# hongsukchoi/Pose2Mesh_RELEASE

Hardware: AMD Instinct MI355X
Metric: SMPL meshes/sec fwd+bwd at batch 256 (higher is better)
Workload: dtype f32 (emulated on the BF16 matrix pipe: every operand as 3 exact bf16 slices = 24-bit significands, 6 slice products per fp32 product, fp32 accumulate)

## Files before the change

pose2mesh_release_amd/csrc/gemm.hip:

```cpp
#include <cstdlib>
#include <type_traits>

#include "p2m_split.h"

namespace p2m {

constexpr int BM = 128;
constexpr int BK = 32;
constexpr int AS_LD = BK + 1;

struct GemmArgs {
  const float* A[3];
  const float* Bm;
  const float* bias;
  const float* addend;
  const float* act_scale;
  const float* act_shift;
  int act_relu;
  int pair_out;
  float* C[3];
  float* stats;
  long M;
  int nplanesA, Ka, a0_shift;
  int N, Nc;
  int ntm, ntn;
  const int* ids;
  int nset, V, tps, compact;
  const float* row_w;
  const unsigned short* Bx;
  int Npad, Ktot;
  const unsigned* a_amax;
  const unsigned* b_amax;
  int a_bits;
  unsigned* amax_out;
  const float* in_scale;
  const float* in_shift;
};

__device__ __forceinline__ bool tile_of_block(int bid, int ntm, int ntn, int& mt, int& nt) {
  int xcd = bid & 7;
  int slot = bid >> 3;
  nt = slot % ntn;
  mt = (slot / ntn) * 8 + xcd;
  return mt < ntm;
}

constexpr int ROWTAB_WORDS = 2 * BM + 2;
__device__ __forceinline__ void rows_weights_fill(const GemmArgs& g, int* rowtab, int i, int t) {
  float* wtab = reinterpret_cast<float*>(rowtab + BM);
  const float w = (i < g.nset) ? g.row_w[i] : 0.f;
  wtab[t] = w;
  float s = w;
#pragma unroll
  for (int o = 32; o > 0; o >>= 1) s += __shfl_xor(s, o);
  if ((t & 63) == 0) wtab[BM + (t >> 6)] = s;
}

template <int BN, bool EXTRA, bool ROWS>
__device__ __forceinline__ void gemm_epilogue(const GemmArgs& g, floatx16 (&acc)[2][BN / 64], float* smem,
                                              const int* rowtab, int mt, long m0, int n0, int rs_i0, int wm, int wn,
                                              int l31, int lhi, int descale = 0) {
  constexpr int WTN = BN / 2;
  constexpr int TN = WTN / 32;
  constexpr int TM = 2;
  float bias_v[TN], sc_v[TN], sh_v[TN];
  int ncol[TN];
#pragma unroll
  for (int j = 0; j < TN; j++) {
    ncol[j] = n0 + wn * WTN + j * 32 + l31;
    bias_v[j] = (g.bias != nullptr && ncol[j] < g.N) ? g.bias[ncol[j]] : 0.f;
    sc_v[j] = (g.act_scale != nullptr && ncol[j] < g.N) ? g.act_scale[ncol[j]] : 1.f;
    sh_v[j] = (g.act_scale != nullptr && ncol[j] < g.N) ? g.act_shift[ncol[j]] : 0.f;
  }
  float csum[TN];
  float vmax = 0.f;
  const bool wst = ROWS && g.row_w != nullptr && g.stats != nullptr;
  const float* wtab = reinterpret_cast<const float*>(rowtab + BM);
#pragma unroll
  for (int j = 0; j < TN; j++) csum[j] = 0.f;
#pragma unroll
  for (int i = 0; i < TM; i++)
#pragma unroll
    for (int j = 0; j < TN; j++) {
      const int n = ncol[j];
      const int q = n / g.Nc;
      const int c = n - q * g.Nc;
      float* Cq = (n < g.N) ? g.C[q] : nullptr;
#pragma unroll
      for (int r = 0; r < 16; r++) {
        const int ml = wm * 64 + i * 32 + (r & 3) + 8 * (r >> 2) + 4 * lhi;
        long row = ROWS ? (long)rowtab[ml] : m0 + ml;
        const bool rok = ROWS ? (row >= 0) : (row < g.M);
        float v = __builtin_ldexpf(acc[i][j][r], descale) + bias_v[j];
        if (g.act_scale != nullptr) v = fmaf(v, sc_v[j], sh_v[j]);
        if (g.act_relu) v = fmaxf(v, 0.f);
        if (EXTRA && g.addend != nullptr && rok && Cq != nullptr) v += g.addend[row * g.N + n];
        acc[i][j][r] = rok ? v : 0.f;
        if (!(EXTRA && g.pair_out) && rok && Cq != nullptr) {
#ifdef P2M_PL_ABL_NOSTORE
          if (v == 12345.678f)
#endif
          Cq[row * g.Nc + c] = v;
          csum[j] += wst ? wtab[ml] * v : v;
          vmax = fmaxf(vmax, amax_abs(v));
        }
        if ((r & 3) == 3) __builtin_amdgcn_sched_barrier(0);
      }
      if (EXTRA && g.pair_out && Cq != nullptr) {
#pragma unroll
        for (int r = 0; r < 16; r += 2) {
          long row = m0 + wm * 64 + i * 32 + (r & 3) + 8 * (r >> 2) + 4 * lhi;
          if (row < g.M) {
            const float pv = acc[i][j][r] + acc[i][j][r + 1];
            Cq[(row >> 1) * g.Nc + c] = pv;
            vmax = fmaxf(vmax, amax_abs(pv));
          }
        }
      }
    }
  if (g.amax_out != nullptr) amax_commit(g.amax_out, vmax);
  if (g.stats == nullptr) return;

  float* red = smem;
  long rows_valid = ROWS ? (long)(g.nset - rs_i0) : g.M - m0;
  if (rows_valid > BM) rows_valid = BM;
#pragma unroll
  for (int j = 0; j < TN; j++) {
    csum[j] += __shfl_xor(csum[j], 32);
    if (lhi == 0) red[wm * BN + wn * WTN + j * 32 + l31] = csum[j];
  }
  __syncthreads();
  float cm2[TN];
#pragma unroll
  for (int j = 0; j < TN; j++) {
    const int cl = wn * WTN + j * 32 + l31;
    const float tot = red[cl] + red[BN + cl];
    const float mean = tot / (wst ? wtab[BM] + wtab[BM + 1] : (float)rows_valid);
    float m2 = 0.f;
#pragma unroll
    for (int i = 0; i < TM; i++)
#pragma unroll
      for (int r = 0; r < 16; r++) {
        const int ml = wm * 64 + i * 32 + (r & 3) + 8 * (r >> 2) + 4 * lhi;
        float d = acc[i][j][r] - mean;
        if (ROWS ? (rowtab[ml] >= 0) : (m0 + ml < g.M)) m2 += wst ? wtab[ml] * d * d : d * d;
      }
    m2 += __shfl_xor(m2, 32);
    cm2[j] = m2;
    csum[j] = tot;
  }
  __syncthreads();
#pragma unroll
  for (int j = 0; j < TN; j++)
    if (lhi == 0) red[wm * BN + wn * WTN + j * 32 + l31] = cm2[j];
  __syncthreads();
  if (wm == 0 && lhi == 0) {
#pragma unroll
    for (int j = 0; j < TN; j++) {
      const int cl = wn * WTN + j * 32 + l31;
      const int n = n0 + cl;
      if (n < g.N) {
        float* st = g.stats + (long)mt * 2 * g.N;
        st[n] = csum[j];
        st[g.N + n] = red[cl] + red[BN + cl];
      }
    }
  }
}

template <int BN, int KB, bool EXTRA, bool ROWS = false>
__global__ __launch_bounds__(256, 2) void k_gemm_planes(GemmArgs g) {
  constexpr int WTN = BN / 2;
  constexpr int TN = WTN / 32;
  constexpr int TM = 2;
  constexpr int LDA = KB + 1;
  constexpr int APASS = BM * KB / 4 / 256;
  constexpr int AROWS = 256 / (KB / 4);
  constexpr int BPASS = KB * BN / 4 / 256;
  constexpr int BROWS = 256 / (BN / 4);
  __shared__ float smem[2 * BM * LDA + 2 * KB * BN + (ROWS ? ROWTAB_WORDS : 0)];
  float* As = smem;
  float* Bs = smem + 2 * BM * LDA;
  int* rowtab = reinterpret_cast<int*>(smem + 2 * BM * LDA + 2 * KB * BN);

  int mt, nt;
  if (!tile_of_block(blockIdx.x, g.ntm, g.ntn, mt, nt)) return;
  const long m0 = (long)mt * BM;
  const int n0 = nt * BN;
  const int t = threadIdx.x;
  const int rs_b = ROWS ? mt / g.tps : 0;
  const int rs_i0 = ROWS ? (mt - rs_b * g.tps) * BM : 0;
  if (ROWS && t < BM) {
    const int i = rs_i0 + t;
    rowtab[t] = (i < g.nset) ? rs_b * g.V + g.ids[i] : -1;
    if (g.row_w != nullptr) rows_weights_fill(g, rowtab, i, t);
  }
  const int lane = t & 63, wave = t >> 6;
  const int wm = wave >> 1, wn = wave & 1;
  const int l31 = lane & 31, lhi = lane >> 5;

  floatx16 acc[TM][TN];
#pragma unroll
  for (int i = 0; i < TM; i++)
#pragma unroll
    for (int j = 0; j < TN; j++)
#pragma unroll
      for (int r = 0; r < 16; r++) acc[i][j][r] = 0.f;

  const int cpp = g.Ka / KB;
  const int nchunks = g.nplanesA * cpp;

  float4 ra[APASS];
  float4 rb[BPASS];
  const int a_row = t / (KB / 4), a_k4 = (t % (KB / 4)) * 4;
  const int b_row = t / (BN / 4), b_c4 = (t % (BN / 4)) * 4;
  long rs_full[ROWS ? APASS : 1], rs_comp[ROWS ? APASS : 1];
  if (ROWS) {
#pragma unroll
    for (int ps = 0; ps < APASS; ps++) {
      const int i = rs_i0 + ps * AROWS + a_row;
      if (i < g.nset) {
        rs_full[ps] = (long)rs_b * g.V + g.ids[i];
        rs_comp[ps] = (long)rs_b * g.nset + i;
      } else {
        rs_full[ps] = -1;
        rs_comp[ps] = -1;
      }
    }
  }

  auto load_chunk = [&](int kc) {
    const int p = kc / cpp;
    const int k0 = (kc - p * cpp) * KB;
    const float* Ap = g.A[p];
    const int sh = (p == 0) ? g.a0_shift : 0;
#pragma unroll
    for (int ps = 0; ps < APASS; ps++) {
      if (ROWS) {
        const long r = (p == 0 || !g.compact) ? rs_full[ps] : rs_comp[ps];
        if (r >= 0)
          ra[ps] = *reinterpret_cast<const float4*>(Ap + (r >> sh) * g.Ka + k0 + a_k4);
        else
          ra[ps] = make_float4(0.f, 0.f, 0.f, 0.f);
      } else {
        long r = m0 + ps * AROWS + a_row;
        if (r < g.M)
          ra[ps] = *reinterpret_cast<const float4*>(Ap + (r >> sh) * g.Ka + k0 + a_k4);
        else
          ra[ps] = make_float4(0.f, 0.f, 0.f, 0.f);
      }
    }
    const float* Bp = g.Bm + (long)(p * g.Ka + k0) * g.N;
#pragma unroll
    for (int ps = 0; ps < BPASS; ps++) {
      int kr = ps * BROWS + b_row;
      int n = n0 + b_c4;
      if (n < g.N)
        rb[ps] = *reinterpret_cast<const float4*>(Bp + (long)kr * g.N + n);
      else
        rb[ps] = make_float4(0.f, 0.f, 0.f, 0.f);
    }
  };
  auto store_chunk = [&](int buf) {
// ... 185 lines not shown
      for (int q = 0; q < NS; q++) *reinterpret_cast<u32x4*>(d + q * BN * LDX) = b[q];
    };
    const int last = n - 1;
#pragma unroll
    for (int i = 0; i < NST; i++) load_chunk(i < last ? i : last, ra[i], rb[i]);
#pragma unroll
    for (int i = 0; i < AHEAD; i++) {
      if (i < n) store_chunk(i, ra[i], rb[i]);
      load_chunk(NST + i < last ? NST + i : last, ra[i], rb[i]);
    }
    lds_barrier();
    int kc = 0;
    for (; kc + (NST - 1) + AHEAD + NST < n; kc += NST) {
#pragma unroll
      for (int i = 0; i < NST; i++) {
        store_chunk(kc + i + AHEAD, ra[(i + AHEAD) % NST], rb[(i + AHEAD) % NST]);
        load_chunk(kc + i + AHEAD + NST, ra[(i + AHEAD) % NST], rb[(i + AHEAD) % NST]);
        lds_barrier();
      }
    }
    for (; kc < n; kc += NST) {
#pragma unroll
      for (int i = 0; i < NST; i++) {
        if (kc + i < n) {
          if (kc + i + AHEAD < n) store_chunk(kc + i + AHEAD, ra[(i + AHEAD) % NST], rb[(i + AHEAD) % NST]);
          if (kc + i + AHEAD + NST < n) load_chunk(kc + i + AHEAD + NST, ra[(i + AHEAD) % NST], rb[(i + AHEAD) % NST]);
          lds_barrier();
        }
      }
    }
  } else {
    frag_t fa[NBUF - 1][NS][TM], fb[NBUF - 1][NS][TN];
    auto read_frags = [&](int kc, frag_t (&a)[NS][TM], frag_t (&b)[NS][TN]) {
      const int buf = kc % NBUF;
      const unsigned short* as = As + buf * A_BUF + (wm * 64 + l31) * LDX + lhi * 8;
      const unsigned short* bs = Bs + buf * B_BUF + (wn * WTN + l31) * LDX + lhi * 8;
#pragma unroll
      for (int sl = 0; sl < NS; sl++) {
#pragma unroll
        for (int i = 0; i < TM; i++)
          a[sl][i] = __builtin_bit_cast(frag_t, *reinterpret_cast<const u32x4*>(as + (sl * BM + i * 32) * LDX));
#pragma unroll
        for (int j = 0; j < TN; j++)
          b[sl][j] = __builtin_bit_cast(frag_t, *reinterpret_cast<const u32x4*>(bs + (sl * BN + j * 32) * LDX));
      }
    };
    auto mfmas = [&](const frag_t (&a)[NS][TM], const frag_t (&b)[NS][TN]) {
#define P2M_PAIR(SA, SB)                                                                       \
  _Pragma("unroll") for (int i = 0; i < TM; i++) _Pragma("unroll") for (int j = 0; j < TN; j++) \
      acc[i][j] = slice_mfma<NS>(a[SA][i], b[SB][j], acc[i][j]);
#ifdef P2M_PL_ABL_NOMFMA
      if constexpr (NS == 3) {
        P2M_PAIR(0, 0)
        for (int sl = 1; sl < NS; sl++)
          for (int i = 0; i < TM; i++) for (int j = 0; j < TN; j++) { asm volatile("" :: "v"(a[sl][i])); asm volatile("" :: "v"(b[sl][j])); }
      } else
#endif
      if constexpr (NS == 3) {
        P2M_PAIR(2, 0)
        P2M_PAIR(0, 2)
        P2M_PAIR(1, 1)
        P2M_PAIR(1, 0)
        P2M_PAIR(0, 1)
        P2M_PAIR(0, 0)
      } else {
        P2M_PAIR(1, 0)
        P2M_PAIR(0, 1)
        P2M_PAIR(0, 0)
      }
#undef P2M_PAIR
    };
    lds_barrier();
    for (int kc = 0; kc < n; kc++) {
      read_frags(kc, fa[0], fb[0]);
      mfmas(fa[0], fb[0]);
      lds_barrier();
    }
  }
  __syncthreads();
  if (!producer) {
    gemm_epilogue<BN, EXTRA, ROWS>(g, acc, smem, rowtab, mt, m0, n0, rs_i0, wm, wn, l31, lhi, descale);
  } else {
    if (g.stats != nullptr) {
      __syncthreads();
      __syncthreads();
      __syncthreads();
    }
  }
}

#ifdef P2M_K1_TRACE
__device__ unsigned long long g_k1_tr[4096][4];
#define P2M_K1T(ev)                                                                      \
  do {                                                                                   \
    if (threadIdx.x == 0 && blockIdx.x < 4096) g_k1_tr[blockIdx.x][ev] = __builtin_amdgcn_s_memtime(); \
  } while (0)
#else
#define P2M_K1T(ev) do { } while (0)
#endif

template <int BN, bool EXTRA, int NS, int KP>
__global__ __launch_bounds__(256, 2) void k_gemm_rows_k1(GemmArgs g) {
  typedef typename SliceFrag<NS>::type frag_t;
  constexpr bool ROWS = true;
  constexpr int WTN = BN / 2;
  constexpr int TN = WTN / 32;
  constexpr int TM = 2;
  constexpr int LDX = KP + 8;
  constexpr int TPR = KP / 4;
  constexpr int RPS = 256 / TPR;
  constexpr int NSW = BM / RPS;
  constexpr int KSTEPS = KP / 16;
  constexpr int A_IMG = NS * BM * LDX;
  static_assert(KP == 64 || KP == 32, "pass width");
  static_assert(A_IMG / 2 >= 2 * BN, "the epilogue's reduction buffer lives in the image");
  __shared__ __attribute__((aligned(16))) float smem[A_IMG / 2 + ROWTAB_WORDS];
  __shared__ __attribute__((aligned(16))) float actco[2 * 256];
  unsigned short* As = reinterpret_cast<unsigned short*>(smem);
  int* rowtab = reinterpret_cast<int*>(smem + A_IMG / 2);

  int mt, nt;
  if (!tile_of_block(blockIdx.x, g.ntm, g.ntn, mt, nt)) return;
  P2M_K1T(0);
  const int t = threadIdx.x;
  const long m0 = (long)mt * BM;
  const int n0 = nt * BN;
  const int rs_b = mt / g.tps;
  const int rs_i0 = (mt - rs_b * g.tps) * BM;
  const int lane = t & 63, wave = t >> 6;
  const int wm = wave >> 1, wn = wave & 1;
  const int l31 = lane & 31, lhi = lane >> 5;
  const int npass = g.Ka / KP;
  const bool in_act = g.in_scale != nullptr;
  const bool live = n0 + wn * WTN < g.N;
  float a_sc = 1.f;
  int descale = 0;
  if (NS == 2) {
    const int sa = slice_scale_exp(*g.a_amax, g.a_bits);
    a_sc = exp2_int(sa);
    descale = -(sa + slice_scale_exp(*g.b_amax, 0));
  }

  int rt_row = -1;
  float rt_w = 0.f, co_sc = 0.f, co_sh = 0.f;
  if (t < BM) {
    const int i = rs_i0 + t;
    if (i < g.nset) {
      rt_row = rs_b * g.V + g.ids[i];
      if (g.row_w != nullptr) rt_w = g.row_w[i];
    }
  }
  if (in_act && t < g.Ka) {
    co_sc = g.in_scale[t];
    co_sh = g.in_shift[t];
  }

  const int a_g = t / TPR;
  const int a_row = KP == 64 ? a_g : (((a_g & 1) << 2) | ((a_g >> 1) & 3) | ((a_g >> 3) << 3));
  const int a_k4 = (t % TPR) * 4;
  const long sbase0 = (((long)rs_b * g.V) >> g.a0_shift) * g.Ka;
  unsigned voff[NSW];
#pragma unroll
  for (int ps = 0; ps < NSW; ps++) {
    int i = rs_i0 + ps * RPS + a_row;
    if (i >= g.nset) i = g.nset - 1;
    voff[ps] = (unsigned)((((g.ids[i] >> g.a0_shift) * g.Ka) + a_k4) * 4);
  }
  f32x4 ra[2][NSW];
  auto load_pass = [&](int p, f32x4 (&a)[NSW]) {
    const char* Ab = reinterpret_cast<const char*>(g.A[0] + sbase0 + p * KP);
#pragma unroll
    for (int ps = 0; ps < NSW; ps++) a[ps] = *reinterpret_cast<const f32x4*>(Ab + voff[ps]);
  };
  auto store_pass = [&](int p, f32x4 (&a)[NSW]) {
    if (in_act) {
      const f32x4 sc = *reinterpret_cast<const f32x4*>(&actco[p * KP + a_k4]);
      const f32x4 sh = *reinterpret_cast<const f32x4*>(&actco[256 + p * KP + a_k4]);
#pragma unroll
      for (int ps = 0; ps < NSW; ps++)
#pragma unroll
        for (int e = 0; e < 4; e++) a[ps][e] = fmaxf(fmaf(a[ps][e], sc[e], sh[e]), 0.f);
    }
#pragma unroll
    for (int ps = 0; ps < NSW; ps++) {
      u32x2 sl[NS];
      split_pack4<NS>(a[ps][0], a[ps][1], a[ps][2], a[ps][3], a_sc, sl);
      unsigned short* d = As + (ps * RPS + a_row) * LDX + a_k4;
#pragma unroll
      for (int q = 0; q < NS; q++) *reinterpret_cast<u32x2*>(d + q * BM * LDX) = sl[q];
    }
  };

  load_pass(0, ra[0]);
  if (npass > 1) load_pass(1, ra[1]);

  const long bx_slice = (long)g.Npad * 16;
  const int nsteps = g.Ka / 16;
  unsigned bx_voff[TN];
// ... 623 lines not shown
    if constexpr (NS == 3) {
      P2M_PAIR(2, 0)
      P2M_PAIR(0, 2)
      P2M_PAIR(1, 1)
      P2M_PAIR(1, 0)
      P2M_PAIR(0, 1)
      P2M_PAIR(0, 0)
    } else {
      P2M_PAIR(1, 0)
      P2M_PAIR(0, 1)
      P2M_PAIR(0, 0)
    }
#undef P2M_PAIR
    P2M_TNT(kc, 2);
    (void)kc;
  };
  auto lds_barrier = [] { asm volatile("s_waitcnt lgkmcnt(0)\n\ts_barrier" ::: "memory"); };

  for (int sb = 0; sb < nsamp; sb++) {
  if (nst > 0) {
    if (producer) {
      load_ids(0, id0);
      load_ids(1, id1);
      load_stage(0, x0, id0, true_type{});
      load_ids(2, id0);
      load_stage(nst > 1 ? 1 : 0, x1, id1, true_type{});
      load_ids(3, id1);
      store_stage(0, 0, x0, true_type{});
      load_stage(nst > 2 ? 2 : nst - 1, x0, id0, true_type{});
      load_ids(4, id0);
      lds_barrier();
      int kc = 0;
      for (; kc + 5 < nst; kc += 2) {
        P2M_TNT(kc + 1, 0);
        store_stage(1, kc + 1, x1, false_type{});
        load_stage(kc + 3, x1, id1, false_type{});
        load_ids(kc + 5, id1);
        P2M_TNT(kc + 1, 3);
        lds_barrier();
        P2M_TNT(kc + 2, 0);
        store_stage(0, kc + 2, x0, false_type{});
        load_stage(kc + 4, x0, id0, false_type{});
        load_ids(kc + 6, id0);
        P2M_TNT(kc + 2, 3);
        lds_barrier();
      }
      for (; kc < nst; kc += 2) {
        if (kc + 1 < nst) store_stage(1, kc + 1, x1, true_type{});
        if (kc + 3 < nst) {
          load_stage(kc + 3, x1, id1, true_type{});
          load_ids(kc + 5, id1);
        }
        lds_barrier();
        if (kc + 1 < nst) {
          if (kc + 2 < nst) store_stage(0, kc + 2, x0, true_type{});
          if (kc + 4 < nst) {
            load_stage(kc + 4, x0, id0, true_type{});
            load_ids(kc + 6, id0);
          }
          lds_barrier();
        }
      }
    } else {
      lds_barrier();
      for (int kc = 0; kc < nst; kc++) {
        P2M_TNT(kc, 0);
        compute(kc & 1, kc);
        P2M_TNT(kc, 3);
        lds_barrier();
      }
    }
  }
  srcb += samp_bytes;
  }
  __syncthreads();

  float* Pc = g.P + (long)chunk * g.Ktot * g.N;
  if (!producer) {
#pragma unroll
    for (int i = 0; i < TM; i++)
#pragma unroll
      for (int j = 0; j < TN; j++) {
        const int n = n0 + wn * WTN + j * 32 + l31;
        float old[16];
#pragma unroll
        for (int r = 0; r < 16; r++) {
          const int krow = kk0 + wm * 64 + i * 32 + (r & 3) + 8 * (r >> 2) + 4 * lhi;
          old[r] = (g.accum && krow < g.Ktot && n < g.N) ? Pc[(long)krow * g.N + n] : 0.f;
        }
#pragma unroll
        for (int r = 0; r < 16; r++) {
          const int krow = kk0 + wm * 64 + i * 32 + (r & 3) + 8 * (r >> 2) + 4 * lhi;
          if (krow < g.Ktot && n < g.N) Pc[(long)krow * g.N + n] = __builtin_ldexpf(acc[i][j][r], descale) + old[r];
        }
      }
  }
  if (kt == 0 && g.Pdb != nullptr) {
    float* red = smem;
    if (producer && !is_a && (st >> 2) < BN / 4) *reinterpret_cast<f32x4*>(red + rq * BN + c4 * 4) = dbs;
    __syncthreads();
    if (t < BN) {
      const float sum = red[t] + red[BN + t] + red[2 * BN + t] + red[3 * BN + t];
      if (n0 + t < g.N) g.Pdb[(long)chunk * g.N + n0 + t] = sum;
    }
  }
}

__global__ void k_naive_gemm_tn(TnArgs g) {
  int o = blockIdx.x * blockDim.x + threadIdx.x;
  const int chunk = blockIdx.y;
  const long r_begin = (long)chunk * g.chunk_rows;
  long r_end = r_begin + g.chunk_rows;
  if (r_end > g.M) r_end = g.M;
  const int nout = g.Ktot * g.N;
  if (o < nout) {
    int kk = o / g.N, n = o - kk * g.N;
    int p = kk / g.Ka, k = kk - p * g.Ka;
    const float* Ap = g.A[p];
    int sh = p == 0 ? g.a0_shift : 0;
    float acc = 0.f;
    const int q = n / g.Gc;
    const float* Gq = g.G[q] + (n - q * g.Gc);
    for (long r = r_begin; r < r_end; r++) acc = fmaf(Ap[(r >> sh) * g.Ka + k], Gq[r * g.Gc], acc);
    g.P[(long)chunk * nout + o] = g.accum ? g.P[(long)chunk * nout + o] + acc : acc;
  }
  if (g.Pdb != nullptr && o < g.N) {
    float s = 0.f;
    const int q = o / g.Gc;
    const float* Gq = g.G[q] + (o - q * g.Gc);
    for (long r = r_begin; r < r_end; r++) s += Gq[r * g.Gc];
    g.Pdb[(long)chunk * g.N + o] = s;
  }
}

__global__ void k_weight_pack(const float* __restrict__ W, float* __restrict__ Wt, float* __restrict__ W2,
                              float* __restrict__ W3, int Fout, int Fin, int K) {
  long idx = (long)blockIdx.x * blockDim.x + threadIdx.x;
  long tot = (long)Fout * Fin * K;
  if (idx >= tot) return;
  int fout = (int)(idx % Fout);
  long kk = idx / Fout;
  int k = (int)(kk / Fin), fin = (int)(kk % Fin);
  float v = W[(long)fout * Fin * K + (long)fin * K + k];
  Wt[idx] = v;
  if (W2) W2[(long)fout * Fin * K + kk] = v;
  if (W3) W3[((long)k * Fout + fout) * Fin + fin] = v;
}

__global__ __launch_bounds__(256) void k_transpose_tiled(const float* __restrict__ W, float* __restrict__ Wt, int R, int C) {
  __shared__ float tile[64][65];
  const int r0 = blockIdx.y * 64, c0 = blockIdx.x * 64;
  const int tq = threadIdx.x & 15, ty = threadIdx.x >> 4;
  const bool vec = (C & 3) == 0 && (R & 3) == 0;
#pragma unroll
  for (int p = 0; p < 4; p++) {
    const int r = r0 + ty + 16 * p, c = c0 + 4 * tq;
    if (r < R) {
      if (vec && c + 3 < C) {
        const float4 v = *reinterpret_cast<const float4*>(W + (long)r * C + c);
        tile[ty + 16 * p][4 * tq] = v.x; tile[ty + 16 * p][4 * tq + 1] = v.y;
        tile[ty + 16 * p][4 * tq + 2] = v.z; tile[ty + 16 * p][4 * tq + 3] = v.w;
      } else {
        for (int e = 0; e < 4; e++)
          if (c + e < C) tile[ty + 16 * p][4 * tq + e] = W[(long)r * C + c + e];
      }
    }
  }
  __syncthreads();
#pragma unroll
  for (int p = 0; p < 4; p++) {
    const int c = c0 + ty + 16 * p, r = r0 + 4 * tq;
    if (c < C) {
      if (vec && r + 3 < R) {
        float4 v;
        v.x = tile[4 * tq][ty + 16 * p]; v.y = tile[4 * tq + 1][ty + 16 * p];
        v.z = tile[4 * tq + 2][ty + 16 * p]; v.w = tile[4 * tq + 3][ty + 16 * p];
// ... 317 lines not shown
extern "C" int p2m_gemm_planes(const float* A0, const float* A1, const float* A2, int32_t nplanesA, int32_t Ka,
                               int32_t a0_shift, const float* Bm, const void* Bsplit, int32_t arith,
                               const void* a_amax, int32_t a_bits, const float* bias,
                               const float* addend, float* C0, float* C1, float* C2, int32_t nplanesC, int32_t Nc,
                               int32_t pair_out, int64_t M, float* stats, const float* act_scale,
                               const float* act_shift, int32_t act_relu, void* amax_out, void* stream) {
  P2M_CHECK_ARG(nplanesA >= 1 && nplanesA <= 3 && nplanesC >= 1 && nplanesC <= 3, "plane count must be 1..3");
  P2M_CHECK_ARG(arith == P2M_ARITH_F32 || arith == P2M_ARITH_BF16X3 || arith == P2M_ARITH_F16X2, "unknown arithmetic");
  P2M_CHECK_ARG((act_scale == nullptr) == (act_shift == nullptr), "act_scale / act_shift must both be given or both NULL");
  P2M_CHECK_ARG(!((act_scale || act_relu) && (stats || pair_out)), "fused activation excludes stats and pair_out");
  P2M_CHECK_ARG(A0 && Bm && C0 && Ka > 0 && Nc > 0, "null pointer or empty shape");
  P2M_CHECK_ARG(a0_shift == 0 || a0_shift == 1, "a0_shift must be 0 or 1");
  if (M <= 0) return P2M_OK;
  GemmArgs g;
  g.A[0] = A0; g.A[1] = A1; g.A[2] = A2;
  g.C[0] = C0; g.C[1] = C1; g.C[2] = C2;
  for (int p = 0; p < nplanesA; p++) P2M_CHECK_ARG(g.A[p] != nullptr, "missing A plane");
  for (int p = 0; p < nplanesC; p++) P2M_CHECK_ARG(g.C[p] != nullptr, "missing C plane");
  P2M_CHECK_ARG((addend == nullptr && !pair_out) || nplanesC == 1, "addend / pair_out need a single output plane");
  P2M_CHECK_ARG(!(pair_out && stats), "pair_out and stats are mutually exclusive");
  g.Bm = Bm; g.bias = bias; g.addend = addend; g.pair_out = pair_out; g.stats = stats; g.M = M;
  g.act_scale = act_scale; g.act_shift = act_shift; g.act_relu = act_relu;
  g.nplanesA = nplanesA; g.Ka = Ka; g.a0_shift = a0_shift;
  g.N = nplanesC * Nc; g.Nc = Nc;
  g.ids = nullptr; g.nset = 0; g.V = 0; g.tps = 0; g.compact = 0; g.row_w = nullptr;
  g.Bx = nullptr; g.Npad = 0; g.Ktot = 0;
  g.a_amax = g.b_amax = nullptr; g.a_bits = 0;
  g.amax_out = static_cast<unsigned*>(amax_out);
  g.in_scale = g.in_shift = nullptr;
  hipStream_t s = (hipStream_t)stream;
  const bool mfma_ok = (Ka % BK == 0) && (g.N % 32 == 0) && (Nc % 32 == 0);
  if (!mfma_ok) {
    P2M_CHECK_ARG(!pair_out, "pair_out needs the MFMA path (Ka % 32 == 0, N % 32 == 0)");
    P2M_CHECK_ARG(!amax_out, "amax_out needs the MFMA path (Ka % 32 == 0, N % 32 == 0)");
    long tot = M * g.N;
    g.ntm = g.ntn = 0;
    hipLaunchKernelGGL(k_naive_gemm_planes, dim3(cdiv(tot, 256)), dim3(256), 0, s, g);
    if (stats) {
      P2M_CHECK_ARG(nplanesC == 1, "stats need a single output plane");
      hipLaunchKernelGGL(k_naive_tile_stats, dim3(cdiv(M, BM)), dim3(64), 0, s, C0, stats, (long)M, g.N);
    }
    return check_launch("gemm_planes(naive)");
  }
  if (arith != P2M_ARITH_F32) {
    P2M_CHECK_ARG(Bsplit != nullptr, "the slice arithmetics need the pre-split weight (p2m_weight_split)");
    P2M_CHECK_ARG(arith != P2M_ARITH_F16X2 || a_amax != nullptr, "P2M_ARITH_F16X2 needs the amax word of the A planes");
    g.Bx = static_cast<const unsigned short*>(Bsplit);
    g.Npad = cdiv(g.N, 128) * 128;
    g.Ktot = nplanesA * Ka;
    if (arith == P2M_ARITH_F16X2) {
      g.a_amax = static_cast<const unsigned*>(a_amax);
      g.a_bits = a_bits;
      g.b_amax = weight_amax_word(Bsplit, arith, g.Npad, g.Ktot);
    }
  }
  g.ntm = cdiv(M, BM);
  launch_gemm_planes<false>(g, addend != nullptr || pair_out, s);
  return check_launch("gemm_planes");
}

extern "C" int p2m_gemm_planes_rows(p2m_graph_t gh, int32_t row_set, int32_t B, const float* A0, const float* A1,
                                    const float* A2, int32_t nplanesA, int32_t Ka, int32_t a0_shift,
                                    int32_t planes_compact, const float* Bm, const void* Bsplit, int32_t arith,
                                    const void* a_amax, int32_t a_bits, const float* bias,
                                    const float* addend, float* C, int32_t N, float* stats, const float* act_scale,
                                    const float* act_shift, int32_t act_relu, void* amax_out, const float* in_scale,
                                    const float* in_shift, void* stream) {
  P2M_CHECK_ARG(gh && A0 && Bm && C, "null pointer");
  P2M_CHECK_ARG((in_scale == nullptr) == (in_shift == nullptr), "in_scale / in_shift must both be given or both NULL");
  P2M_CHECK_ARG(in_scale == nullptr || (arith != P2M_ARITH_F32 && Ka <= 256),
                "activation on load exists in the slice arithmetics only, for Ka <= 256");
  P2M_CHECK_ARG(arith == P2M_ARITH_F32 || arith == P2M_ARITH_BF16X3 || arith == P2M_ARITH_F16X2, "unknown arithmetic");
  P2M_CHECK_ARG(arith == P2M_ARITH_F32 || Bsplit != nullptr, "the slice arithmetics need the pre-split weight (p2m_weight_split)");
  P2M_CHECK_ARG(arith != P2M_ARITH_F16X2 || a_amax != nullptr, "P2M_ARITH_F16X2 needs the amax word of the A planes");
  P2M_CHECK_ARG((act_scale == nullptr) == (act_shift == nullptr), "act_scale / act_shift must both be given or both NULL");
  P2M_CHECK_ARG(!((act_scale || act_relu) && stats), "fused activation excludes stats");
  P2M_CHECK_ARG(row_set_valid(row_set), "row_set must be 1 (real), 2 (fake), 3 (paired real) or 4 (paired fake)");
  P2M_CHECK_ARG(nplanesA >= 1 && nplanesA <= 3, "plane count must be 1..3");
  P2M_CHECK_ARG(Ka > 0 && Ka % BK == 0 && N > 0 && N % 32 == 0, "Ka and N must be positive multiples of 32");
  P2M_CHECK_ARG(a0_shift == 0 || a0_shift == 1, "a0_shift must be 0 or 1");
  const Graph& gr = *reinterpret_cast<const Graph*>(gh);
  const RowSet rs = row_set_of(gr, row_set);
  if (B <= 0 || rs.n == 0) return P2M_OK;
  GemmArgs g;
  g.A[0] = A0; g.A[1] = A1; g.A[2] = A2;
  for (int p = 0; p < nplanesA; p++) P2M_CHECK_ARG(g.A[p] != nullptr, "missing A plane");
  g.C[0] = C; g.C[1] = nullptr; g.C[2] = nullptr;
  g.Bm = Bm; g.bias = bias; g.addend = addend; g.pair_out = 0; g.stats = stats;
  g.act_scale = act_scale; g.act_shift = act_shift; g.act_relu = act_relu;
  g.nplanesA = nplanesA; g.Ka = Ka; g.a0_shift = a0_shift; g.N = N; g.Nc = N;
  g.ids = rs.ids; g.nset = rs.n; g.V = rs.V; g.tps = cdiv(rs.n, BM); g.compact = planes_compact;
  g.row_w = (stats != nullptr && row_set == 2) ? gr.fake_wts : nullptr;
  g.Bx = arith == P2M_ARITH_F32 ? nullptr : static_cast<const unsigned short*>(Bsplit);
  g.Npad = cdiv(N, 128) * 128;
  g.Ktot = nplanesA * Ka;
  g.a_amax = g.b_amax = nullptr; g.a_bits = 0;
  if (arith == P2M_ARITH_F16X2) {
    g.a_amax = static_cast<const unsigned*>(a_amax);
    g.a_bits = a_bits;
    g.b_amax = weight_amax_word(Bsplit, arith, g.Npad, g.Ktot);
  }
  g.amax_out = static_cast<unsigned*>(amax_out);
  g.in_scale = in_scale; g.in_shift = in_shift;
  g.M = (long)B * g.tps * BM;
  g.ntm = B * g.tps;
  launch_gemm_planes<true>(g, addend != nullptr, (hipStream_t)stream);
  return check_launch("gemm_planes_rows");
}

extern "C" int32_t p2m_rows_tiles_per_sample(p2m_graph_t gh, int32_t row_set) {
  if (!gh || !row_set_valid(row_set)) return 0;
  const Graph& gr = *reinterpret_cast<const Graph*>(gh);
  return cdiv(row_set_of(gr, row_set).n, BM);
}

static int gemm_tn_impl(const float* A0, const float* A1, const float* A2, int32_t nplanesA, int32_t Ka,
                        int32_t a0_shift, const float* G0, const float* G1, const float* G2, int32_t nplanesG,
                        int32_t Gc, int64_t M, int64_t chunk_rows, float* P, float* Pdb, int32_t arith,
                        const void* a_amax, int32_t a_bits, const void* g_amax, int32_t g_bits, int32_t accumulate,
                        void* stream);
extern "C" int p2m_gemm_tn(const float* A0, const float* A1, const float* A2, int32_t nplanesA, int32_t Ka,
                           int32_t a0_shift, const float* G0, const float* G1, const float* G2, int32_t nplanesG,
                           int32_t Gc, int64_t M, int64_t chunk_rows, float* P, float* Pdb, int32_t arith,
                           const void* a_amax, int32_t a_bits, const void* g_amax, int32_t g_bits, void* stream) {
  return gemm_tn_impl(A0, A1, A2, nplanesA, Ka, a0_shift, G0, G1, G2, nplanesG, Gc, M, chunk_rows, P, Pdb, arith, a_amax,
                      a_bits, g_amax, g_bits, 0, stream);
}
extern "C" int p2m_gemm_tn_acc(const float* A, int32_t Ka, const float* G, int32_t N, int64_t M, float* P, int32_t arith,
                               const void* a_amax, const void* g_amax, void* stream) {
  const int64_t chunk_rows = ((M + 31) / 32) * 32;
  return gemm_tn_impl(A, nullptr, nullptr, 1, Ka, 0, G, nullptr, nullptr, 1, N, M, chunk_rows > 0 ? chunk_rows : 32, P,
                      nullptr, arith, a_amax, 0, g_amax, 0, 1, stream);
}
static int gemm_tn_impl(const float* A0, const float* A1, const float* A2, int32_t nplanesA, int32_t Ka,
                        int32_t a0_shift, const float* G0, const float* G1, const float* G2, int32_t nplanesG,
                        int32_t Gc, int64_t M, int64_t chunk_rows, float* P, float* Pdb, int32_t arith,
                        const void* a_amax, int32_t a_bits, const void* g_amax, int32_t g_bits, int32_t accumulate,
                        void* stream) {
  P2M_CHECK_ARG(nplanesA >= 1 && nplanesA <= 3 && nplanesG >= 1 && nplanesG <= 3, "plane count must be 1..3");
  P2M_CHECK_ARG(arith == P2M_ARITH_F32 || arith == P2M_ARITH_BF16X3 || arith == P2M_ARITH_F16X2, "unknown arithmetic");
  P2M_CHECK_ARG(arith != P2M_ARITH_F16X2 || (a_amax && g_amax), "P2M_ARITH_F16X2 needs the amax words of both operands");
  const int N = nplanesG * Gc;
  P2M_CHECK_ARG(A0 && G0 && P && Ka > 0 && Gc > 0 && chunk_rows > 0, "null pointer or empty shape");
  P2M_CHECK_ARG(a0_shift == 0 || a0_shift == 1, "a0_shift must be 0 or 1");
  if (M <= 0) return P2M_OK;
  TnArgs g;
  g.A[0] = A0; g.A[1] = A1; g.A[2] = A2;
  for (int p = 0; p < nplanesA; p++) P2M_CHECK_ARG(g.A[p] != nullptr, "missing A plane");
  g.G[0] = G0; g.G[1] = G1; g.G[2] = G2; g.Gc = Gc;
  for (int p = 0; p < nplanesG; p++) P2M_CHECK_ARG(g.G[p] != nullptr, "missing G plane");
  g.P = P; g.Pdb = Pdb; g.M = M; g.chunk_rows = chunk_rows;
  g.nplanesA = nplanesA; g.Ka = Ka; g.a0_shift = a0_shift; g.Ktot = nplanesA * Ka; g.N = N;
  g.ids = nullptr; g.nset = 0; g.V = 0; g.splits = 1; g.compact = 0;
  g.a_amax = static_cast<const unsigned*>(a_amax); g.g_amax = static_cast<const unsigned*>(g_amax);
  g.a_bits = a_bits; g.g_bits = g_bits;
  g.a_scale = g.a_shift = nullptr;
  const int nchunks = cdiv(M, chunk_rows);
  g.nchunks = nchunks;
  g.accum = accumulate;
  P2M_CHECK_ARG(!accumulate || nchunks == 1, "accumulation needs the whole reduction in one chunk");
  hipStream_t s = (hipStream_t)stream;
  const bool mfma_ok = (Ka % 4 == 0) && (N % 32 == 0) && (Gc % 4 == 0) && (g.Ktot >= 32);
  if (!mfma_ok) {
    g.nkt = g.ntn = 0;
    int nout = g.Ktot * N;
    if (nout < N) nout = N;
// ... 133 lines not shown
```

Measured before the change: 6248.

## Restructure GEMM epilogue with 32-bit offsets, prefetched addends and fewer barriers

Rewrites the GEMM epilogue to work in groups of four rows. Row offsets come from a vectorised rowtab read and are held as 32-bit byte offsets from a per-sample base pointer. Addend loads are double-buffered one group ahead, waves whose column range lies entirely outside N skip the work, and the stats reduction uses two separate LDS buffers so one barrier is dropped. The TN kernel also skips the old-value reload when not accumulating. In exchange, pointer offsets are limited to 32 bits (enforced by a new argument check), register pressure rises from copying the accumulators into val, and the producer barrier count must stay matched to the consumer's.

Measured after the change: 6447 (median of 6 runs). +3.2%, better.

```diff
diff --git a/pose2mesh_release_amd/csrc/gemm.hip b/pose2mesh_release_amd/csrc/gemm.hip
--- a/pose2mesh_release_amd/csrc/gemm.hip
+++ b/pose2mesh_release_amd/csrc/gemm.hip
@@ -56,6 +56,19 @@
   if ((t & 63) == 0) wtab[BM + (t >> 6)] = s;
 }
 
+template <bool ROWS>
+__device__ __forceinline__ void epi_group_rows(const int* rowtab, long m0, long M, int ml0, int (&rl)[4]) {
+  if (ROWS) {
+    const u32x4 rt = *reinterpret_cast<const u32x4*>(rowtab + ml0);
+#pragma unroll
+    for (int e = 0; e < 4; e++) rl[e] = (int)rt[e];
+  } else {
+#pragma unroll
+    for (int e = 0; e < 4; e++) rl[e] = (m0 + ml0 + e < M) ? ml0 + e : -1;
+  }
+}
+
+constexpr int EPI_BARRIERS = 2;
 template <int BN, bool EXTRA, bool ROWS>
 __device__ __forceinline__ void gemm_epilogue(const GemmArgs& g, floatx16 (&acc)[2][BN / 64], float* smem,
                                               const int* rowtab, int mt, long m0, int n0, int rs_i0, int wm, int wn,
@@ -63,109 +76,214 @@
   constexpr int WTN = BN / 2;
   constexpr int TN = WTN / 32;
   constexpr int TM = 2;
-  float bias_v[TN], sc_v[TN], sh_v[TN];
-  int ncol[TN];
-#pragma unroll
-  for (int j = 0; j < TN; j++) {
-    ncol[j] = n0 + wn * WTN + j * 32 + l31;
-    bias_v[j] = (g.bias != nullptr && ncol[j] < g.N) ? g.bias[ncol[j]] : 0.f;
-    sc_v[j] = (g.act_scale != nullptr && ncol[j] < g.N) ? g.act_scale[ncol[j]] : 1.f;
-    sh_v[j] = (g.act_scale != nullptr && ncol[j] < g.N) ? g.act_shift[ncol[j]] : 0.f;
-  }
+  constexpr int NG = TM * 4;
+  const int wnu = __builtin_amdgcn_readfirstlane(wn);
+  const bool live = n0 + wnu * WTN < g.N;
+  const bool wst = ROWS && g.row_w != nullptr && g.stats != nullptr;
+  const float* wtab = reinterpret_cast<const float*>(rowtab + BM);
+  const int mlw = wm * 64 + 4 * lhi;
   float csum[TN];
   float vmax = 0.f;
-  const bool wst = ROWS && g.row_w != nullptr && g.stats != nullptr;
-  const float* wtab = reinterpret_cast<const float*>(rowtab + BM);
 #pragma unroll
   for (int j = 0; j < TN; j++) csum[j] = 0.f;
+  float val[TM][TN][16];
 #pragma unroll
   for (int i = 0; i < TM; i++)
 #pragma unroll
+    for (int j = 0; j < TN; j++)
+#pragma unroll
+      for (int r = 0; r < 16; r++) val[i][j][r] = acc[i][j][r];
+
+  if (live) {
+    float bias_v[TN], sc_v[TN], sh_v[TN];
+    bool cok[TN];
+    unsigned c4[TN];
+    char* Cb[TN];
+    const bool pair = EXTRA && !ROWS && g.pair_out;
+    const long rowbase = ROWS ? (long)(mt / g.tps) * g.V : m0;
+    const int rowbase32 = (int)rowbase;
+    const unsigned pitch = (unsigned)g.Nc * 4u;
+#pragma unroll
     for (int j = 0; j < TN; j++) {
-      const int n = ncol[j];
-      const int q = n / g.Nc;
-      const int c = n - q * g.Nc;
-      float* Cq = (n < g.N) ? g.C[q] : nullptr;
-#pragma unroll
-      for (int r = 0; r < 16; r++) {
-        const int ml = wm * 64 + i * 32 + (r & 3) + 8 * (r >> 2) + 4 * lhi;
-        long row = ROWS ? (long)rowtab[ml] : m0 + ml;
-        const bool rok = ROWS ? (row >= 0) : (row < g.M);
-        float v = __builtin_ldexpf(acc[i][j][r], descale) + bias_v[j];
-        if (g.act_scale != nullptr) v = fmaf(v, sc_v[j], sh_v[j]);
-        if (g.act_relu) v = fmaxf(v, 0.f);
-        if (EXTRA && g.addend != nullptr && rok && Cq != nullptr) v += g.addend[row * g.N + n];
-        acc[i][j][r] = rok ? v : 0.f;
-        if (!(EXTRA && g.pair_out) && rok && Cq != nullptr) {
+      const int nu = n0 + wnu * WTN + j * 32;
+      const int n = nu + l31;
+      cok[j] = n < g.N;
+      bias_v[j] = (g.bias != nullptr && cok[j]) ? g.bias[n] : 0.f;
+      sc_v[j] = (g.act_scale != nullptr && cok[j]) ? g.act_scale[n] : 1.f;
+      sh_v[j] = (g.act_scale != nullptr && cok[j]) ? g.act_shift[n] : 0.f;
+      const int q = (nu >= g.Nc ? 1 : 0) + (nu >= 2 * g.Nc ? 1 : 0);
+      float* const Cq = q == 0 ? g.C[0] : (q == 1 ? g.C[1] : g.C[2]);
+      Cb[j] = reinterpret_cast<char*>(Cq + (pair ? rowbase >> 1 : rowbase) * g.Nc);
+      c4[j] = (unsigned)(n - q * g.Nc) * 4u;
+    }
+    const char* const Ab = reinterpret_cast<const char*>(g.addend + (EXTRA && g.addend != nullptr ? rowbase * g.Nc : 0));
+    constexpr unsigned NOROW = 0xFFFFFFFFu;
+
+    auto row_offsets = [&](int gi, unsigned (&ro)[4]) {
+      int rl[4];
+      epi_group_rows<ROWS>(rowtab, m0, g.M, mlw + (gi >> 2) * 32 + (gi & 3) * 8, rl);
+#pragma unroll
+      for (int e = 0; e < 4; e++) {
+        ro[e] = rl[e] >= 0 ? (unsigned)(ROWS ? rl[e] - rowbase32 : rl[e]) * pitch : NOROW;
+        asm volatile("" : "+v"(ro[e]));
+      }
+    };
+    auto walk = [&](auto add_tag, auto keep_tag) {
+      constexpr bool ADD = decltype(add_tag)::value;
+      constexpr bool KEEP = decltype(keep_tag)::value;
+      float ad[2][ADD ? TN : 1][4];
+      auto fetch = [&](int gi) {
+        unsigned ro[4];
+        row_offsets(gi, ro);
+#pragma unroll
+        for (int e = 0; e < 4; e++) {
+          const unsigned lo = ro[e] != NOROW ? ro[e] : 0u;
+#pragma unroll
+          for (int j = 0; j < TN; j++)
+            ad[gi & 1][j][e] = *reinterpret_cast<const float*>(Ab + (lo + (cok[j] ? c4[j] : 0u)));
+        }
+      };
+      if constexpr (ADD) fetch(0);
+#pragma unroll
+      for (int j = 0; j < TN; j++) asm volatile("" : "+v"(bias_v[j]), "+v"(sc_v[j]), "+v"(sh_v[j]));
+#pragma unroll
+      for (int gi = 0; gi < NG; gi++) {
+        const int i = gi >> 2, r0 = (gi & 3) * 4;
+        const int ml0 = mlw + i * 32 + (gi & 3) * 8;
+        if constexpr (ADD) {
+          if (gi + 1 < NG) fetch(gi + 1);
+        }
+        __builtin_amdgcn_sched_barrier(0);
+        unsigned ro[4];
+        row_offsets(gi, ro);
+        float vg[TN][4];
+#pragma unroll
+        for (int e = 0; e < 4; e++) {
+          const int r = r0 + e;
+          const bool rok = ro[e] != NOROW;
+#pragma unroll
+          for (int j = 0; j < TN; j++) {
+            float v = __builtin_ldexpf(val[i][j][r], descale) + bias_v[j];
+            if (g.act_scale != nullptr) v = fmaf(v, sc_v[j], sh_v[j]);
+            if (g.act_relu) v = fmaxf(v, 0.f);
+            if constexpr (ADD) v += ad[gi & 1][j][e];
+            asm volatile("" : "+v"(v));
+            vg[j][e] = v;
+            if constexpr (KEEP) val[i][j][r] = v;
+            if (!pair && rok && cok[j]) {
 #ifdef P2M_PL_ABL_NOSTORE
-          if (v == 12345.678f)
+              if (v == 12345.678f)
 #endif
-          Cq[row * g.Nc + c] = v;
-          csum[j] += wst ? wtab[ml] * v : v;
-          vmax = fmaxf(vmax, amax_abs(v));
-        }
-        if ((r & 3) == 3) __builtin_amdgcn_sched_barrier(0);
-      }
-      if (EXTRA && g.pair_out && Cq != nullptr) {
-#pragma unroll
-        for (int r = 0; r < 16; r += 2) {
-          long row = m0 + wm * 64 + i * 32 + (r & 3) + 8 * (r >> 2) + 4 * lhi;
-          if (row < g.M) {
-            const float pv = acc[i][j][r] + acc[i][j][r + 1];
-            Cq[(row >> 1) * g.Nc + c] = pv;
-            vmax = fmaxf(vmax, amax_abs(pv));
+              *reinterpret_cast<float*>(Cb[j] + (ro[e] + c4[j])) = v;
+            }
           }
         }
-      }
-    }
+        if (pair) {
+#pragma unroll
+          for (int e = 0; e < 4; e += 2) {
+            if (m0 + ml0 + e < g.M) {
+#pragma unroll
+              for (int j = 0; j < TN; j++)
+                if (cok[j]) {
+                  const float pv = vg[j][e] + (m0 + ml0 + e + 1 < g.M ? vg[j][e + 1] : 0.f);
+                  *reinterpret_cast<float*>(Cb[j] + ((unsigned)((ml0 + e) >> 1) * pitch + c4[j])) = pv;
+                  vmax = fmaxf(vmax, amax_abs(pv));
+                }
+            }
+          }
+        } else {
+          f32x4 w4 = {0.f, 0.f, 0.f, 0.f};
+          if (KEEP && wst) w4 = *reinterpret_cast<const f32x4*>(wtab + ml0);
+#pragma unroll
+          for (int e = 0; e < 4; e++)
+#pragma unroll
+            for (int j = 0; j < TN; j++) {
+              const float v = vg[j][e];
+              const bool ok = ro[e] != NOROW && cok[j];
+              if constexpr (KEEP) {
+                const float term = wst ? w4[e] * v : v;
+                csum[j] += ok ? term : 0.f;
+              }
+              vmax = fmaxf(vmax, ok ? amax_abs(v) : 0.f);
+            }
+        }
+#pragma unroll
+        for (int j = 0; j < TN; j++) asm volatile("" : "+v"(csum[j]));
+        asm volatile("" : "+v"(vmax));
+        __builtin_amdgcn_sched_barrier(0);
+      }
+    };
+    const bool add = EXTRA && g.addend != nullptr;
+    if (g.stats != nullptr) {
+      if (add) walk(std::true_type{}, std::true_type{});
+      else walk(std::false_type{}, std::true_type{});
+    } else {
+      if (add) walk(std::true_type{}, std::false_type{});
+      else walk(std::false_type{}, std::false_type{});
+    }
+  }
+
+  if (g.stats != nullptr) {
+    float* red = smem;
+    float* red2 = smem + 2 * BN;
+    long rows_valid = ROWS ? (long)(g.nset - rs_i0) : g.M - m0;
+    if (rows_valid > BM) rows_valid = BM;
+    if (live) {
+#pragma unroll
+      for (int j = 0; j < TN; j++) {
+        csum[j] += __shfl_xor(csum[j], 32);
+        if (lhi == 0) red[wm * BN + wn * WTN + j * 32 + l31] = csum[j];
+      }
+    }
+    __syncthreads();
+    if (live) {
+      float mean[TN], m2[TN];
+#pragma unroll
+      for (int j = 0; j < TN; j++) {
+        const int cl = wn * WTN + j * 32 + l31;
+        const float tot = red[cl] + red[BN + cl];
+        mean[j] = tot / (wst ? wtab[BM] + wtab[BM + 1] : (float)rows_valid);
+        m2[j] = 0.f;
+        csum[j] = tot;
+      }
+#pragma unroll
+      for (int gi = 0; gi < NG; gi++) {
+        const int i = gi >> 2, r0 = (gi & 3) * 4;
+        const int ml0 = mlw + i * 32 + (gi & 3) * 8;
+        int rl[4];
+        epi_group_rows<ROWS>(rowtab, m0, g.M, ml0, rl);
+        f32x4 w4 = {0.f, 0.f, 0.f, 0.f};
+        if (wst) w4 = *reinterpret_cast<const f32x4*>(wtab + ml0);
+#pragma unroll
+        for (int e = 0; e < 4; e++)
+#pragma unroll
+          for (int j = 0; j < TN; j++) {
+            const float d = val[i][j][r0 + e] - mean[j];
+            const float wd = wst ? w4[e] * d : d;
+            m2[j] = rl[e] >= 0 ? fmaf(wd, d, m2[j]) : m2[j];
+          }
+      }
+#pragma unroll
+      for (int j = 0; j < TN; j++) {
+        m2[j] += __shfl_xor(m2[j], 32);
+        if (lhi == 0) red2[wm * BN + wn * WTN + j * 32 + l31] = m2[j];
+      }
+    }
+    __syncthreads();
+    if (live && wm == 0 && lhi == 0) {
+#pragma unroll
+      for (int j = 0; j < TN; j++) {
+        const int cl = wn * WTN + j * 32 + l31;
+        const int n = n0 + cl;
+        if (n < g.N) {
+          float* st = g.stats + (long)mt * 2 * g.N;
+          st[n] = csum[j];
+          st[g.N + n] = red2[cl] + red2[BN + cl];
+        }
+      }
+    }
+  }
   if (g.amax_out != nullptr) amax_commit(g.amax_out, vmax);
-  if (g.stats == nullptr) return;
-
-  float* red = smem;
-  long rows_valid = ROWS ? (long)(g.nset - rs_i0) : g.M - m0;
-  if (rows_valid > BM) rows_valid = BM;
-#pragma unroll
-  for (int j = 0; j < TN; j++) {
-    csum[j] += __shfl_xor(csum[j], 32);
-    if (lhi == 0) red[wm * BN + wn * WTN + j * 32 + l31] = csum[j];
-  }
-  __syncthreads();
-  float cm2[TN];
-#pragma unroll
-  for (int j = 0; j < TN; j++) {
-    const int cl = wn * WTN + j * 32 + l31;
-    const float tot = red[cl] + red[BN + cl];
-    const float mean = tot / (wst ? wtab[BM] + wtab[BM + 1] : (float)rows_valid);
-    float m2 = 0.f;
-#pragma unroll
-    for (int i = 0; i < TM; i++)
-#pragma unroll
-      for (int r = 0; r < 16; r++) {
-        const int ml = wm * 64 + i * 32 + (r & 3) + 8 * (r >> 2) + 4 * lhi;
-        float d = acc[i][j][r] - mean;
-        if (ROWS ? (rowtab[ml] >= 0) : (m0 + ml < g.M)) m2 += wst ? wtab[ml] * d * d : d * d;
-      }
-    m2 += __shfl_xor(m2, 32);
-    cm2[j] = m2;
-    csum[j] = tot;
-  }
-  __syncthreads();
-#pragma unroll
-  for (int j = 0; j < TN; j++)
-    if (lhi == 0) red[wm * BN + wn * WTN + j * 32 + l31] = cm2[j];
-  __syncthreads();
-  if (wm == 0 && lhi == 0) {
-#pragma unroll
-    for (int j = 0; j < TN; j++) {
-      const int cl = wn * WTN + j * 32 + l31;
-      const int n = n0 + cl;
-      if (n < g.N) {
-        float* st = g.stats + (long)mt * 2 * g.N;
-        st[n] = csum[j];
-        st[g.N + n] = red[cl] + red[BN + cl];
-      }
-    }
-  }
 }
 
 template <int BN, int KB, bool EXTRA, bool ROWS = false>
@@ -178,7 +296,7 @@
   constexpr int AROWS = 256 / (KB / 4);
   constexpr int BPASS = KB * BN / 4 / 256;
   constexpr int BROWS = 256 / (BN / 4);
-  __shared__ float smem[2 * BM * LDA + 2 * KB * BN + (ROWS ? ROWTAB_WORDS : 0)];
+  __shared__ __attribute__((aligned(16))) float smem[2 * BM * LDA + 2 * KB * BN + (ROWS ? ROWTAB_WORDS : 0)];
   float* As = smem;
   float* Bs = smem + 2 * BM * LDA;
   int* rowtab = reinterpret_cast<int*>(smem + 2 * BM * LDA + 2 * KB * BN);
@@ -530,9 +648,8 @@
     gemm_epilogue<BN, EXTRA, ROWS>(g, acc, smem, rowtab, mt, m0, n0, rs_i0, wm, wn, l31, lhi, descale);
   } else {
     if (g.stats != nullptr) {
-      __syncthreads();
-      __syncthreads();
-      __syncthreads();
+#pragma unroll
+      for (int b = 0; b < EPI_BARRIERS; b++) __syncthreads();
     }
   }
 }
@@ -561,7 +678,7 @@
   constexpr int KSTEPS = KP / 16;
   constexpr int A_IMG = NS * BM * LDX;
   static_assert(KP == 64 || KP == 32, "pass width");
-  static_assert(A_IMG / 2 >= 2 * BN, "the epilogue's reduction buffer lives in the image");
+  static_assert(A_IMG / 2 >= 4 * BN, "the epilogue's two reduction buffers live in the image");
   __shared__ __attribute__((aligned(16))) float smem[A_IMG / 2 + ROWTAB_WORDS];
   __shared__ __attribute__((aligned(16))) float actco[2 * 256];
   unsigned short* As = reinterpret_cast<unsigned short*>(smem);
@@ -1351,16 +1468,24 @@
 #pragma unroll
       for (int j = 0; j < TN; j++) {
         const int n = n0 + wn * WTN + j * 32 + l31;
-        float old[16];
-#pragma unroll
-        for (int r = 0; r < 16; r++) {
-          const int krow = kk0 + wm * 64 + i * 32 + (r & 3) + 8 * (r >> 2) + 4 * lhi;
-          old[r] = (g.accum && krow < g.Ktot && n < g.N) ? Pc[(long)krow * g.N + n] : 0.f;
-        }
-#pragma unroll
-        for (int r = 0; r < 16; r++) {
-          const int krow = kk0 + wm * 64 + i * 32 + (r & 3) + 8 * (r >> 2) + 4 * lhi;
-          if (krow < g.Ktot && n < g.N) Pc[(long)krow * g.N + n] = __builtin_ldexpf(acc[i][j][r], descale) + old[r];
+        if (g.accum) {
+          float old[16];
+#pragma unroll
+          for (int r = 0; r < 16; r++) {
+            const int krow = kk0 + wm * 64 + i * 32 + (r & 3) + 8 * (r >> 2) + 4 * lhi;
+            old[r] = (krow < g.Ktot && n < g.N) ? Pc[(long)krow * g.N + n] : 0.f;
+          }
+#pragma unroll
+          for (int r = 0; r < 16; r++) {
+            const int krow = kk0 + wm * 64 + i * 32 + (r & 3) + 8 * (r >> 2) + 4 * lhi;
+            if (krow < g.Ktot && n < g.N) Pc[(long)krow * g.N + n] = __builtin_ldexpf(acc[i][j][r], descale) + old[r];
+          }
+        } else {
+#pragma unroll
+          for (int r = 0; r < 16; r++) {
+            const int krow = kk0 + wm * 64 + i * 32 + (r & 3) + 8 * (r >> 2) + 4 * lhi;
+            if (krow < g.Ktot && n < g.N) Pc[(long)krow * g.N + n] = __builtin_ldexpf(acc[i][j][r], descale) + 0.f;
+          }
         }
       }
   }
@@ -1844,6 +1969,7 @@
   const Graph& gr = *reinterpret_cast<const Graph*>(gh);
   const RowSet rs = row_set_of(gr, row_set);
   if (B <= 0 || rs.n == 0) return P2M_OK;
+  P2M_CHECK_ARG((long)rs.V * N < (1l << 30), "one sample of C must stay below 4 GiB (V * N < 2^30)");
   GemmArgs g;
   g.A[0] = A0; g.A[1] = A1; g.A[2] = A2;
   for (int p = 0; p < nplanesA; p++) P2M_CHECK_ARG(g.A[p] != nullptr, "missing A plane");
```
